# Desperodoo/distributed_multi_agent_reinforcement_learning

Measured on AMD Instinct MI355X. Metric: env-steps/sec (whole node), pursuit-evasion 8-agent 4096-env, higher is better.
Workload: dtype f64 environment / f32 policy (f32 matrix products evaluated from exact 3-way bf16 operand splits, f32 accumulation and storage)

## Files before the change

### distributed_multi_agent_reinforcement_learning_amd/csrc/mappo_ops.hip

```cpp
#include <hip/hip_runtime.h>
#include <stdint.h>
#include <stdlib.h>
#include <string.h>

#include <mutex>

#include "mappo_ops.h"
#include "mappo_ops_diag.h"
#include "sb_common.hpp"
#include "sb_wgrad.hpp"

namespace {

constexpr int MAX_P = 16;

__device__ __forceinline__ float msg_dot4(const float *w, const float4 &qv) {
    return __builtin_fmaf(w[3], qv.w, __builtin_fmaf(w[2], qv.z, __builtin_fmaf(w[1], qv.y, w[0] * qv.x)));
}

struct MsgDims {
    int R, P, K, E, din, q_div, adj_mode, rpb;
    int64_t p_rs, q_rs, e_rs, adj_rs, o_is;
};

// ... 750 lines not shown
    stats[2] = mean;
    stats[3] = sqrt(var > 0.0 ? var : 0.0);
}

__global__ __launch_bounds__(256) void k_gae_center(int64_t n, const float *adv, double *stats) {
    const double mean = stats[2];
    double d = 0.0, unused = 0.0;
    for (int64_t i = (int64_t)blockIdx.x * 256 + threadIdx.x; i < n; i += (int64_t)gridDim.x * 256) {
        const double x = (double)adv[i] - mean;
        d += x * x;
    }
    gae_block_sum(d, unused);
    if (threadIdx.x == 0) stats[4 + 2 * blockIdx.x] = d;
}

__global__ void k_gae_std(int64_t n, int nblk, double *stats) {
    double d = 0.0;
    for (int b = 0; b < nblk; b++) d += stats[4 + 2 * b];
    stats[1] = d;
    stats[3] = sqrt(d / (double)(n - 1));
}

__global__ void k_gae_norm(int64_t n, float *adv, const float *active, const double *stats) {
    const int64_t i = (int64_t)blockIdx.x * blockDim.x + threadIdx.x;
    if (i < n) {
        const float mean = (float)stats[2], sd = (float)stats[3];
        adv[i] = (adv[i] - mean) / (sd + 1e-5f) * active[i];
    }
}

__global__ void k_advance_counter(uint64_t *ctr, uint64_t by) { *ctr += by; }

constexpr int SN_MAX_A = 16, SN_MAX_H = 1024;
__global__ __launch_bounds__(256) void k_sn_power(int A, int H, const float *__restrict__ W, float *u, float *v, float eps, int n_iter,
                                                  float *__restrict__ w_eff) {
    __shared__ float s_u[SN_MAX_A], s_s[SN_MAX_A], s_v[SN_MAX_H], s_red[4];
    const int tid = threadIdx.x, lane = tid & 63, wave = tid >> 6;
    if (tid < A) s_u[tid] = u[tid];
    for (int k = tid; k < H; k += 256) s_v[k] = v[k];
    __syncthreads();
    for (int it = 0; it <= n_iter; it++) {
        if (it > 0) {
            float part = 0.f;
            for (int k = tid; k < H; k += 256) {
                float t = 0.f;
                for (int a = 0; a < A; a++) t = __builtin_fmaf(W[(size_t)a * H + k], s_u[a], t);
                s_v[k] = t;
                part = __builtin_fmaf(t, t, part);
            }
            for (int off = 32; off > 0; off >>= 1) part += __shfl_xor(part, off);
            if (lane == 0) s_red[wave] = part;
            __syncthreads();
            const float den = fmaxf(sqrtf((s_red[0] + s_red[1]) + (s_red[2] + s_red[3])), eps);
            for (int k = tid; k < H; k += 256) s_v[k] = s_v[k] / den;
            __syncthreads();
        }
        for (int a = wave; a < A; a += 4) {
            float part = 0.f;
            for (int k = lane; k < H; k += 64) part = __builtin_fmaf(W[(size_t)a * H + k], s_v[k], part);
            for (int off = 32; off > 0; off >>= 1) part += __shfl_xor(part, off);
            if (lane == 0) s_s[a] = part;
        }
        __syncthreads();
        if (it > 0) {
            if (tid == 0) {
                float q = 0.f;
                for (int a = 0; a < A; a++) q = __builtin_fmaf(s_s[a], s_s[a], q);
                const float den = fmaxf(sqrtf(q), eps);
                for (int a = 0; a < A; a++) s_u[a] = s_s[a] / den;
            }
            __syncthreads();
        }
    }
    float sigma = 0.f;
    for (int a = 0; a < A; a++) sigma = __builtin_fmaf(s_u[a], s_s[a], sigma);
    for (int i = tid; i < A * H; i += 256) w_eff[i] = W[i] / sigma;
    if (n_iter > 0) {
        if (tid < A) u[tid] = s_u[tid];
        for (int k = tid; k < H; k += 256) v[k] = s_v[k];
    }
}

__device__ __forceinline__ void philox4x32_10(uint32_t c0, uint32_t c1, uint32_t c2, uint32_t c3, uint32_t k0, uint32_t k1, uint32_t *o) {
    for (int i = 0; i < 10; i++) {
        const uint64_t p0 = (uint64_t)0xD2511F53u * c0, p1 = (uint64_t)0xCD9E8D57u * c2;
        const uint32_t n0 = (uint32_t)(p1 >> 32) ^ c1 ^ k0, n1 = (uint32_t)p1, n2 = (uint32_t)(p0 >> 32) ^ c3 ^ k1, n3 = (uint32_t)p0;
        c0 = n0; c1 = n1; c2 = n2; c3 = n3;
        k0 += 0x9E3779B9u; k1 += 0xBB67AE85u;
    }
    o[0] = c0; o[1] = c1; o[2] = c2; o[3] = c3;
}

__global__ void k_categorical(int R, int A, const float *probs, uint64_t seed, uint64_t offset, const uint64_t *offset_dev, int greedy,
                              int32_t *action, float *logp) {
    const int r = blockIdx.x * blockDim.x + threadIdx.x;
    if (r >= R) return;
    if (offset_dev) offset += *offset_dev;
    const float *p = probs + (size_t)r * A;
    float tot = 0.f;
    for (int k = 0; k < A; k++) tot += p[k];
    int a = 0;
    if (greedy) {
        float best = p[0];
        for (int k = 1; k < A; k++) if (p[k] > best) { best = p[k]; a = k; }
    } else {
        uint32_t o[4];
        const uint64_t ctr = offset + (uint64_t)r;
        philox4x32_10((uint32_t)ctr, (uint32_t)(ctr >> 32), 0u, 0u, (uint32_t)seed, (uint32_t)(seed >> 32), o);
// ... 3 lines not shown
        for (int k = 0; k < A; k++) {
            cum += p[k];
            if (p[k] > 0.f) a = k;
            if (u < cum) break;
        }
    }
    action[r] = a;
    if (logp) {
        float pn = p[a] / tot;
        pn = fminf(fmaxf(pn, 1.1920929e-07f), 1.f - 1.1920929e-07f);
        logp[r] = logf(pn);
    }
}


__device__ __forceinline__ void wave_fence() {
    __builtin_amdgcn_fence(__ATOMIC_RELEASE, "wavefront");
    __builtin_amdgcn_wave_barrier();
    __builtin_amdgcn_fence(__ATOMIC_ACQUIRE, "wavefront");
}

template <int CTRL>
__device__ __forceinline__ float dpp_f(float v) { return __int_as_float(__builtin_amdgcn_update_dpp(0, __float_as_int(v), CTRL, 0xF, 0xF, true)); }
__device__ __forceinline__ float row16_sum(float v) {
    v += dpp_f<0xB1>(v);
    v += dpp_f<0x4E>(v);
    v += dpp_f<0x141>(v);
    v += dpp_f<0x140>(v);
    return v;
}

constexpr int HEAD_MAX_A = 16, HEAD_H = 128;
template <bool SAMPLE, int AT>
__global__ __launch_bounds__(256) void k_head(int R, int A, const float *__restrict__ feat, const float *__restrict__ W, const float *__restrict__ b,
                                              float *__restrict__ y, uint64_t seed, uint64_t *counter, unsigned int *done, int greedy,
                                              int32_t *__restrict__ action, float *__restrict__ logp) {
    __shared__ float s_y[4][64][AT + 1];
    const int lane = threadIdx.x & 63, wave = threadIdx.x >> 6, nw = (gridDim.x * blockDim.x) >> 6;
    const int i = lane & 15, g = lane >> 4;
    float w[AT][8];
#pragma unroll
    for (int a = 0; a < AT; a++)
#pragma unroll
        for (int k = 0; k < 8; k++) w[a][k] = W[a * HEAD_H + 8 * i + k];
    const uint64_t offset = SAMPLE ? *counter : 0ull;
    float (*sy)[AT + 1] = s_y[wave];
    for (int r0 = (blockIdx.x * 4 + wave) * 64; r0 < R; r0 += nw * 64) {
        float4 fall[16][2];
#pragma unroll
        for (int st = 0; st < 16; st++) {
            const int r = r0 + 4 * st + g;
            fall[st][0] = fall[st][1] = make_float4(0.f, 0.f, 0.f, 0.f);
            if (r < R) {
                fall[st][0] = *(const float4 *)(feat + (size_t)r * HEAD_H + 8 * i);
                fall[st][1] = *(const float4 *)(feat + (size_t)r * HEAD_H + 8 * i + 4);
            }
        }
#pragma unroll
        for (int st = 0; st < 16; st++) {
            const int row = 4 * st + g;
            const float4 fa = fall[st][0], fb = fall[st][1];
            float mine = 0.f;
#pragma unroll
            for (int a = 0; a < AT; a++) {
                float sum = fa.x * w[a][0];
                sum = __builtin_fmaf(fa.y, w[a][1], sum); sum = __builtin_fmaf(fa.z, w[a][2], sum); sum = __builtin_fmaf(fa.w, w[a][3], sum);
                sum = __builtin_fmaf(fb.x, w[a][4], sum); sum = __builtin_fmaf(fb.y, w[a][5], sum); sum = __builtin_fmaf(fb.z, w[a][6], sum);
                sum = __builtin_fmaf(fb.w, w[a][7], sum);
                sum = row16_sum(sum);
                mine = i == a ? sum : mine;
            }
            if (i < AT) sy[row][i] = mine;
        }
        wave_fence();
        const int r = r0 + lane;
        if (r < R) {
            float v[AT];
#pragma unroll
            for (int a = 0; a < AT; a++) v[a] = sy[lane][a] + b[a];
// ... 11 lines not shown
#pragma unroll
                for (int a = 0; a < AT; a++) { p[a] = p[a] / den; tot += p[a]; }
                int act = 0;
                float pa = p[0];
                if (greedy) {
#pragma unroll
                    for (int a = 1; a < AT; a++) { const bool up = p[a] > pa; pa = up ? p[a] : pa; act = up ? a : act; }
                } else {
                    uint32_t o[4];
                    const uint64_t ctr = offset + (uint64_t)r;
                    philox4x32_10((uint32_t)ctr, (uint32_t)(ctr >> 32), 0u, 0u, (uint32_t)seed, (uint32_t)(seed >> 32), o);
                    const float u = ((float)(o[0] >> 8) + 0.5f) * (1.0f / 16777216.0f) * tot;
                    float cum = 0.f;
                    bool found = false;
                    act = AT - 1;
                    pa = p[AT - 1];
#pragma unroll
                    for (int a = 0; a < AT; a++) {
                        cum += p[a];
                        const bool take = !found && p[a] > 0.f;
                        act = take ? a : act;
                        pa = take ? p[a] : pa;
                        found = found || u < cum;
                    }
                }
                action[r] = act;
                float pn = pa / tot;
                pn = fminf(fmaxf(pn, 1.1920929e-07f), 1.f - 1.1920929e-07f);
                logp[r] = logf(pn);
            }
        }
        wave_fence();
    }
    if (SAMPLE) {
        __syncthreads();
        if (threadIdx.x == 0) {
            __threadfence();
            if (atomicAdd(done, 1u) == gridDim.x - 1) {
                *counter = offset + (uint64_t)R;
                *done = 0u;
                __threadfence();
            }
        }
    }
}

__device__ __forceinline__ float sigmoidf_(float x) { return 1.f / (1.f + expf(-x)); }
__device__ __forceinline__ float sigmoid_hw(float x) { return __builtin_amdgcn_rcpf(1.f + __expf(-x)); }
__device__ __forceinline__ float tanh_hw(float x) { return 1.f - 2.f * __builtin_amdgcn_rcpf(1.f + __expf(2.f * x)); }

__global__ void k_gru_gates_fwd(int B, int H, const float *gi, const float *gh, const float *bhh, const float *hprev, float *hout,
                                float *save ) {
    const int idx = blockIdx.x * blockDim.x + threadIdx.x;
    const int H4 = H >> 2;
    if (idx >= B * H4) return;
    const int b = idx / H4, c = (idx - b * H4) << 2;
    const float4 gir = *(const float4 *)(gi + (size_t)b * 3 * H + c), giz = *(const float4 *)(gi + (size_t)b * 3 * H + H + c),
                 gin = *(const float4 *)(gi + (size_t)b * 3 * H + 2 * H + c);
    const float4 ghr = *(const float4 *)(gh + (size_t)b * 3 * H + c), ghz = *(const float4 *)(gh + (size_t)b * 3 * H + H + c),
                 ghn = *(const float4 *)(gh + (size_t)b * 3 * H + 2 * H + c);
    const float4 br = *(const float4 *)(bhh + c), bz = *(const float4 *)(bhh + H + c), bn = *(const float4 *)(bhh + 2 * H + c);
    const float4 hp = *(const float4 *)(hprev + (size_t)b * H + c);
    float4 r, z, n, hn, ho;
#define GRU_ONE(f)                                  \
    r.f = sigmoidf_(gir.f + ghr.f + br.f);          \
    z.f = sigmoidf_(giz.f + ghz.f + bz.f);          \
    hn.f = ghn.f + bn.f;                            \
    n.f = tanhf(gin.f + r.f * hn.f);                \
    ho.f = (1.f - z.f) * n.f + z.f * hp.f;
    GRU_ONE(x) GRU_ONE(y) GRU_ONE(z) GRU_ONE(w)
#undef GRU_ONE
    *(float4 *)(hout + (size_t)b * H + c) = ho;
    if (save) {
        const size_t BH = (size_t)B * H, o = (size_t)b * H + c;
        *(float4 *)(save + o) = r; *(float4 *)(save + BH + o) = z; *(float4 *)(save + 2 * BH + o) = n; *(float4 *)(save + 3 * BH + o) = hn;
    }
// ... 1307 lines not shown

int head_grid(int R) { const int g = (R + 255) / 256; return g < 1024 ? g : 1024; }

int head_linear(int32_t R, int32_t A, int32_t H, const float *feat, const float *W, const float *b, float *y, void *stream) {
    if (R < 0 || A < 1 || A > HEAD_MAX_A || H != HEAD_H || !feat || !W || !b || !y || ((uintptr_t)feat & 15)) return MO_ERR_BAD_ARG;
    if (R == 0) return 0;
    hipStream_t st = (hipStream_t)stream;
#define HEAD_LIN(AT) case AT: hipLaunchKernelGGL((k_head<false, AT>), dim3(head_grid(R)), dim3(256), 0, st, R, A, feat, W, b, y, (uint64_t)0, \
                                       (uint64_t *)nullptr, (unsigned int *)nullptr, 0, (int32_t *)nullptr, (float *)nullptr); break;
    switch (A) {
        HEAD_LIN(1) HEAD_LIN(2) HEAD_LIN(3) HEAD_LIN(4) HEAD_LIN(5) HEAD_LIN(6) HEAD_LIN(7) HEAD_LIN(8) HEAD_LIN(9) HEAD_LIN(10) HEAD_LIN(11)
        HEAD_LIN(12) HEAD_LIN(13) HEAD_LIN(14) HEAD_LIN(15) HEAD_LIN(16)
    }
#undef HEAD_LIN
    return (int)hipGetLastError();
}

int head_sample(int32_t R, int32_t A, int32_t H, const float *feat, const float *W, const float *b, uint64_t seed, uint64_t *counter,
                uint32_t *ticket, int32_t greedy, int32_t *action, float *logp, void *stream) {
    if (R < 0 || A < 1 || A > HEAD_MAX_A || H != HEAD_H || !feat || !W || !b || !counter || !ticket || !action || !logp || ((uintptr_t)feat & 15))
        return MO_ERR_BAD_ARG;
    if (R == 0) return 0;
    hipStream_t st = (hipStream_t)stream;
#define HEAD_SMP(AT) case AT: hipLaunchKernelGGL((k_head<true, AT>), dim3(head_grid(R)), dim3(256), 0, st, R, A, feat, W, b, (float *)nullptr, seed, \
                                       counter, ticket, (int)greedy, action, logp); break;
    switch (A) {
        HEAD_SMP(1) HEAD_SMP(2) HEAD_SMP(3) HEAD_SMP(4) HEAD_SMP(5) HEAD_SMP(6) HEAD_SMP(7) HEAD_SMP(8) HEAD_SMP(9) HEAD_SMP(10) HEAD_SMP(11)
        HEAD_SMP(12) HEAD_SMP(13) HEAD_SMP(14) HEAD_SMP(15) HEAD_SMP(16)
    }
#undef HEAD_SMP
    return (int)hipGetLastError();
}

int gru_gates_fwd(int32_t B, int32_t H, const float *gi, const float *gh, const float *b_hh, const float *h_prev, float *h_out,
                  float *save, void *stream) {
    if (B < 1 || H < 4 || (H & 3) || !gi || !gh || !b_hh || !h_prev || !h_out) return MO_ERR_BAD_ARG;
    const int n = B * (H >> 2);
    hipLaunchKernelGGL(k_gru_gates_fwd, dim3((n + 255) / 256), dim3(256), 0, (hipStream_t)stream, B, H, gi, gh, b_hh, h_prev, h_out, save);
    return (int)hipGetLastError();
}

int gru_gates_bwd(int32_t B, int32_t H, const float *dout, const float *dcarry, const float *save, const float *h_prev, float *dgi,
                  float *dgh, float *dh_direct, void *stream) {
    if (B < 1 || H < 4 || (H & 3) || !save || !h_prev || !dgi || !dgh || !dh_direct) return MO_ERR_BAD_ARG;
    const int n = B * (H >> 2);
    hipLaunchKernelGGL(k_gru_gates_bwd, dim3((n + 255) / 256), dim3(256), 0, (hipStream_t)stream, B, H, dout, dcarry, save, h_prev, dgi, dgh,
                       dh_direct);
    return (int)hipGetLastError();
}

int gru_cell_fwd_multi(int32_t n_nets, const mo_gru_cell_net *nets, int32_t B, int32_t H, void *stream) {
    if (n_nets < 1 || n_nets > MO_GRU_CELL_MAX_NETS || !nets || B < 1 || H != GRU_H) return MO_ERR_BAD_ARG;
    GruCellNets a;
    memset(&a, 0, sizeof a);
    for (int k = 0; k < n_nets; k++) {
        const mo_gru_cell_net &m = nets[k];
        if (!m.x || !m.h_prev || !m.w_ih || !m.w_hh || !m.b_ih || !m.b_hh || !m.h_out) return MO_ERR_BAD_ARG;
        if (((uintptr_t)m.x & 15) || ((uintptr_t)m.h_prev & 15) || ((uintptr_t)m.w_ih & 15) || ((uintptr_t)m.w_hh & 15)) return MO_ERR_BAD_ARG;
        a.n[k] = m;
    }
    const int nblk = (B + GRU_RB - 1) / GRU_RB;
    int dev = 0, cus = 256;
    if (hipGetDevice(&dev) == hipSuccess && hipDeviceGetAttribute(&cus, hipDeviceAttributeMultiprocessorCount, dev) != hipSuccess) cus = 256;
    int per = cus / n_nets;
    if (per < 1) per = 1;
    const int grid = nblk < per ? nblk : per;
// ... 284 lines not shown
```

### distributed_multi_agent_reinforcement_learning_amd/mappo.py

```python
import contextlib
import gc
import logging
import threading
import types

import numpy as np
import torch

from . import ops
from .model import build_actor_critic, pair_embeddings, pair_heads, sequence_forward_pair
from .pe_env import status_or, status_text

_log = logging.getLogger(__name__)

BUFFER_KEYS = ("p_state", "e_state", "o_state", "p_adj", "e_adj", "o_adj", "actor_historical_embedding",
               "critic_historical_embedding", "v_n", "a_n", "a_logprob_n", "r", "active")


class _Buffer(dict):

    def __missing__(self, key):
        if key == "o_adj" and "o_adj_bits" in self:
            v = ops.unpack_adj_bits(self["o_adj_bits"], self.num_obstacle_slots)
            self[key] = v
# ... 404 lines not shown
        _gc_depth += 1
    try:
        yield
    finally:
        with _gc_lock:
            _gc_depth -= 1
            if _gc_depth == 0 and _gc_was_on:
                gc.enable()


class _RolloutState:

    def __init__(self, agent, env):
        self.agent = agent
        N, P = env.num_envs, env.num_defender
        O = env.pe_cfg.O
        d, L, H, E = agent.depth, agent.num_layers, agent.rnn_hidden_dim, agent.embedding_dim
        dev = agent.device
        self.N, self.P, self.d = N, P, d
        z = lambda *s: torch.zeros(s, dtype=torch.float32, device=dev)
        self.obs = dict(p_state=z(N, P, 4), e_state=z(N, 1, 4), p_adj=z(N, P, P), e_adj=z(N, P, 1),
                        o_adj_bits=torch.zeros((N, P, ops.adj_row_words(O)), dtype=torch.int32, device=dev))
        self.o_state = z(N, O, 4)
        self.o_kvalid = torch.zeros(N, dtype=torch.int32, device=dev)
        self.hbuf_a, self.hbuf_c = z(2, L, N * P, H), z(2, L, N * P, H)
        self.quirk = bool(agent.reference_quirks and agent.actor.shared_net is agent.critic.shared_net)
        self.M = ((d + 1) // 2 if self.quirk else d) + 1
        self.ring = z(self.M, 2, N, P, E)
        self.t = 0
        self.a_n = torch.zeros((N, P), dtype=torch.int32, device=dev)
        self.logp, self.v, self.raw = z(N, P), z(N, P), z(N, P)
        self.counter = torch.full((1,), int(agent.sample_rank) << 40, dtype=torch.int64, device=dev)
        self.ticket = torch.zeros(1, dtype=torch.int32, device=dev)
        self.period = self.M if self.M % 2 == 0 else 2 * self.M
        self.graphs = {}
        self.pair_forward = agent.actor.shared_net is agent.critic.shared_net
        ops.gemm_workspace(dev)

    @property
    def ha(self):
        return self.hbuf_a[self.t & 1]

    @property
    def hc(self):
        return self.hbuf_c[self.t & 1]

    @property
    def a_cur(self):
        return self.ring[(self.t - 1) % self.M][0]

    @property
    def c_cur(self):
        return self.ring[(self.t - 1) % self.M][1]

    @property
    def hist_c(self):
        return None if self.quirk else self.ring[:, 1]

    def reset(self, env):
        for t in (self.hbuf_a, self.hbuf_c, self.ring):
            t.zero_()
        self.t = 0
        self.o_state.copy_(env.boundary_map.obstacle_agent)
        self.o_kvalid.copy_(env.n_obs)

    def _obs(self):
        o = dict(self.obs)
        o["o_state"], o["o_kvalid"] = self.o_state, self.o_kvalid
        return o

    def _hops(self, t):
        d, M, ring = self.d, self.M, self.ring
        if self.quirk:
            hops = [ring[(t - 1 - j // 2) % M][1 - j % 2] for j in range(d)]
            return hops, hops
        return [ring[(t - 1 - k) % M][0] for k in range(d)], [ring[(t - 1 - k) % M][1] for k in range(d)]

    def policy_step(self, forced_actions=None):
        ag = self.agent
        hops_a, hops_c = self._hops(self.t)
        slot = self.ring[self.t % self.M]
        a_cur, c_cur = slot[0], slot[1]
        o = self._obs()
        ha_cur, hc_cur = self.ha, self.hc
        ha_new, hc_new = self.hbuf_a[(self.t + 1) & 1], self.hbuf_c[(self.t + 1) & 1]
        if self.pair_forward and not torch.is_grad_enabled():
            emb = ag.actor.shared_net.forward_pair(o["p_state"], o["e_state"], o["o_state"], o["p_adj"], o["e_adj"], o["o_adj_bits"],
                                                   hops_a, hops_c, o["o_kvalid"], 1, slot)
            a_emb, c_emb = emb[0], emb[1]
            if ag.actor.use_rnn and ag.critic.use_rnn:
                E = a_emb.shape[-1]
                fa, fc = ops.gru_step_multi([a_emb.reshape(-1, E), c_emb.reshape(-1, E)], [ha_cur, hc_cur], [ag.actor.GRU, ag.critic.GRU],
                                            hiddens_out=[ha_new, hc_new])
                feat_a, feat_c = fa.reshape(self.N, self.P, -1), fc.reshape(self.N, self.P, -1)
                ha, hc = ha_new, hc_new
            else:
                feat_a, ha = ag.actor._rollout_features(a_emb, ha_cur, True)
                feat_c, hc = ag.critic._rollout_features(c_emb, hc_cur, True)
            v = ag.critic.head(feat_c, out=self.v)
            w_a = ag.actor.head_weight() if forced_actions is None else None
            feat_a = feat_a.contiguous()
            if w_a is not None and ops._head_ok(feat_a, w_a, ag.actor.Mean.bias):
                ops.head_sample(feat_a, w_a, ag.actor.Mean.bias, ag.sample_seed, self.counter, self.ticket, (self.a_n, self.logp))
                prob = None
            else:
                prob = torch.softmax(ag.actor.head(feat_a), dim=-1)
        else:
            prob, ha, a_emb = ag.actor(o, hops_a, ha_cur, 0, inplace_hidden=True, emb_out=a_cur)
            v, hc, c_emb = ag.critic(o, hops_c, hc_cur, 0, rollout=True, inplace_hidden=True, emb_out=c_cur)
        if forced_actions is not None:
            self.a_n.copy_(forced_actions.to(torch.int32))
            self.logp.copy_(torch.distributions.Categorical(probs=prob).log_prob(forced_actions))
        elif prob is not None:
            ops.categorical_sample(prob, ag.sample_seed, 0, counter=self.counter, out=(self.a_n, self.logp))
        if ha is not ha_new:
            ha_new.copy_(ha)
        if hc is not hc_new:
            hc_new.copy_(hc)
        if a_emb.data_ptr() != a_cur.data_ptr():
            a_cur.copy_(a_emb)
        if c_emb.data_ptr() != c_cur.data_ptr():
            c_cur.copy_(c_emb)
        if v.data_ptr() != self.v.data_ptr():
            self.v.copy_(v.reshape(self.N, self.P))

    def step(self, forced_actions=None):
        self.policy_step(forced_actions)
        self.t += 1

    def value_step(self):
        ag, d, t, M = self.agent, self.d, self.t, self.M
        hops = []
        if d:
            if self.quirk:
                hops = ([self.ring[(t - 1) % M][1]] + self._hops(t - 1)[1])[:d]
            else:
                hops = self._hops(t)[1]
        v, hc, c_emb = ag.critic(self._obs(), hops, self.hc, 0, rollout=True)
        self.v.copy_(v.reshape(self.N, self.P))

    def replay_policy_step(self):
        phase = self.t % self.period
        g = self.graphs.get(phase)
        if g is None:
            g = self.graphs[phase] = self._capture()
        g.replay()
        self.t += 1

    def _capture(self):
        live = (self.hbuf_a, self.hbuf_c, self.ring, self.counter, self.a_n, self.logp, self.v)
        keep = [t.clone() for t in live]
        side = torch.cuda.Stream()
        side.wait_stream(torch.cuda.current_stream())
        with torch.cuda.stream(side):
            for _ in range(2):
                self.policy_step()
        torch.cuda.current_stream().wait_stream(side)
        g = torch.cuda.CUDAGraph()
        with _collector_paused():
            with torch.cuda.graph(g, capture_error_mode="thread_local"):
                self.policy_step()
        for t, k in zip(live, keep):
            t.copy_(k)
        return g
```

### distributed_multi_agent_reinforcement_learning_amd/model.py

```python
import torch
import torch.nn as nn
import torch.nn.functional as F
from torch.nn.utils import spectral_norm
from torch.nn.utils.spectral_norm import SpectralNorm

from . import ops


class HeadLinear(nn.Linear):

    def forward(self, x):
        return ops.linear_skinny(x, self.weight, self.bias)


def _ortho_linear(n_in, n_out, cls=nn.Linear):
    layer = cls(n_in, n_out)
    for name, param in layer.named_parameters():
        if "bias" in name:
            nn.init.constant_(param, 0)
        elif "weight" in name:
            nn.init.orthogonal_(param, gain=1.0)
    return layer


# ... 128 lines not shown
                h = cats[k + 1][..., E:]
            else:
                h = out if out is not None else torch.empty((2, R, P, E), dtype=p.dtype, device=p.device)
            cat_2d, h_2d = cats[k].view(2 * R * P, 2 * E), ops.block2d(h)
            if ops.split_linear_ok(cat_2d, fk.weight, h_2d):
                ops.split_linear(cat_2d, fk.weight, fk.bias, True, out=h_2d)
            else:
                ops.gemm_nt(cat_2d, fk.weight, fk.bias, True, out=h_2d)
        return h


def _o_adj(obs):
    return obs["o_adj_bits"] if "o_adj_bits" in obs else obs["o_adj"]


class _Trunk(nn.Module):
    use_rnn = True

    def _rollout_features(self, embedding, hidden_state, inplace_hidden=False):
        R, P, E = embedding.shape
        if not self.use_rnn:
            return embedding, hidden_state
        feat, hidden_state = ops.gru(embedding.reshape(1, R * P, E), hidden_state, self.GRU, inplace_hidden)
        return feat.reshape(R, P, self.rnn_hidden_dim), hidden_state

    def _sequence_features(self, embedding, batch, steps):
        P = embedding.shape[1]
        if not self.use_rnn:
            return embedding.reshape(batch, steps, P, self.rnn_input_dim).permute(1, 0, 2, 3)
        h0 = torch.zeros(self.num_layers, batch * P, self.rnn_hidden_dim, dtype=embedding.dtype, device=embedding.device)
        feat, _ = ops.gru(embedding.reshape(batch * steps * P, self.rnn_input_dim), h0, self.GRU, agents=P, steps=steps)
        return feat.reshape(steps, batch, P, self.rnn_hidden_dim)

    def head_weight(self):
        m = self.Mean
        if torch.is_grad_enabled() or not m.bias.is_cuda:
            return None
        hooks = list(m._forward_pre_hooks.values())
        if not hooks:
            return m.weight
        if (len(hooks) == 1 and isinstance(hooks[0], SpectralNorm) and hooks[0].name == "weight" and hooks[0].dim == 0 and m.weight_orig.dim() == 2
                and m.weight_orig.shape[0] <= 16 and m.weight_orig.shape[1] <= 1024):
            return ops.spectral_norm_weight(m.weight_orig, m.weight_u, m.weight_v, hooks[0].eps,
                                            hooks[0].n_power_iterations if m.training else 0)
        return None

    def head(self, feat, out=None):
        w = self.head_weight()
        if w is None:
            y = self.Mean(feat)
            return y if out is None else out.copy_(y.reshape(out.shape))
        return ops.head_linear(feat, w, self.Mean.bias, out=out)

    def get_weights(self):
        return {k: v.cpu() for k, v in self.state_dict().items()}

    def set_weights(self, weights):
        self.load_state_dict(weights)

    def get_gradients(self):
        return [None if p.grad is None else p.grad.data.cpu().numpy() for p in self.parameters()]

    def set_gradients(self, gradients, device):
        for g, p in zip(gradients, self.parameters()):
            if g is not None:
                p.grad = torch.as_tensor(g).to(device)


class SharedActor(_Trunk):
    def __init__(self, shared_net, rnn_input_dim, action_dim, num_layers, rnn_hidden_dim, is_sn=False):
        super().__init__()
        self.shared_net = shared_net
        self.num_layers = num_layers
        self.rnn_input_dim = rnn_input_dim
        self.rnn_hidden_dim = rnn_hidden_dim
        self.GRU = nn.GRU(rnn_input_dim, rnn_hidden_dim, num_layers)
        self.Mean = _make_linear(rnn_hidden_dim, action_dim, is_sn, HeadLinear)

# ... 150 lines not shown
```

### distributed_multi_agent_reinforcement_learning_amd/ops.py

```python
import ctypes as C
import os

import torch
import torch.nn.functional as F

from . import build as _build

ADJ_TENSOR, ADJ_ONES, ADJ_VALID, ADJ_BITS = 0, 1, 2, 3
EXPORTS = ("dhgn_msg_agg_fwd", "dhgn_msg_agg3_fwd", "dhgn_msg_agg_bwd", "dhgn_msg_agg_bwd_workspace", "dhgn_msg_agg_ones_sorted_ok", "dhgn_msg_agg_ones_sorted_fwd",
           "dhgn_msg_agg_ones_sorted_bwd", "dhgn_msg_agg_ones_sorted_workspace", "gae_advnorm", "gae_advnorm_workspace", "categorical_sample",
           "categorical_sample_counter",
           "gru_gates_fwd", "gru_gates_bwd", "gru_cell_fwd", "gru_cell_fwd_multi", "gru_cell_split_fwd_multi", "sb_gemm_n128", "sb_gemm", "gru_seq_fwd", "gru_seq_fwd_multi", "gru_seq_split_fwd_multi", "gru_seq_split_bwd_multi", "gru_seq_save_elems", "gru_seq_bwd", "gru_seq_bwd_multi", "gru_seq_bwd_workspace", "wgrad_tn", "wgrad_tn_workspace", "wgrad_split_tn", "wgrad_split_tn2", "wgrad_split_workspace", "rollout_record", "ppo_loss_fwd_bwd", "ppo_loss_prob_fwd_bwd", "ppo_loss_workspace",
           "gauss_head_sample", "ppo_loss_gauss_fwd_bwd", "ppo_loss_gauss_workspace", "gauss_head_sample_ex", "ppo_loss_gauss_ex_fwd_bwd",
           "ppo_loss_gauss_ex_workspace", "mappo_ops_error_string")

_lib = None


def lib_path():
    return _build.lib_path("libmappo_ops.so")


def load_library():
    global _lib
    if _lib is None:
        path = lib_path()
        if not os.path.exists(path):
            raise RuntimeError(f"{path} is missing: build it with __graft_entry__.build() (hipcc --offload-arch=gfx950); "
                               "the fused MAPPO ops have no fallback")
        L = C.CDLL(path)
        vp, i32, i64, f32 = C.c_void_p, C.c_int32, C.c_int64, C.c_float
        L.dhgn_msg_agg_fwd.argtypes = [i32, i32, i32, i32, i32, vp, i64, vp, i64, i32, vp, i64, vp, i64, i32, vp, vp, vp, vp, i64, vp]
        L.dhgn_msg_agg_bwd.argtypes = [i32, i32, i32, i32, i32, vp, i64, vp, i64, i32, vp, i64, vp, i64, i32, vp, vp, vp, vp, i64, vp, vp, vp, vp]
        L.dhgn_msg_agg3_fwd.argtypes = [vp, i32, i32, i32, vp, i64, vp, i64, vp]
        L.dhgn_msg_agg3_pair_fwd.argtypes = [vp, i32, i32, i32, vp, i64, vp, vp, vp, i64, vp]
        L.dhgn_msg_agg3_pair01_fwd.argtypes = [vp, i32, i32, i32, vp, i64, vp, vp, i64, vp]
        L.dhgn_msg_agg_bwd_pair.argtypes = [i32, i32, i32, i32, i32, vp, i64, vp, i64, i32, vp, i64, vp, i64, vp, vp, vp, vp, i64, vp, vp, vp, vp]
        L.dhgn_msg_agg3_pair_pos_fwd.argtypes = [vp, i32, i32, i32, vp, i64, vp, vp, vp, i64, vp, i64, vp, vp, vp, i64, vp]
        L.spectral_norm_weight.argtypes = [i32, i32, vp, vp, vp, f32, i32, vp, vp]
        L.dhgn_msg_agg_bwd_workspace.argtypes = [i32, i32]
        L.dhgn_msg_agg_bwd_workspace.restype = i64
        L.dhgn_msg_agg_ones_sorted_ok.argtypes = [i32] * 6
        L.dhgn_msg_agg_ones_sorted_workspace.argtypes = [i32, i32, i32, i32, i32, vp, vp, vp]
        L.dhgn_msg_agg_ones_sorted_workspace.restype = i64
        L.dhgn_msg_agg_ones_sorted_fwd.argtypes = [i32, i32, i32, i32, vp, i64, vp, i64, i32, vp, vp, vp, i64, vp, vp, vp]
        L.dhgn_msg_agg_ones_sorted_bwd.argtypes = [i32, i32, i32, i32, vp, i64, i32, vp, i64, vp, vp, vp, vp, vp, vp]
        L.gae_advnorm.argtypes = [i32, i32, i32, vp, vp, vp, f32, f32, i32, vp, vp, vp, vp]
        L.gae_advnorm_workspace.restype = i64
        L.categorical_sample.argtypes = [i32, i32, vp, C.c_uint64, C.c_uint64, i32, vp, vp, vp]
        L.categorical_sample_counter.argtypes = [i32, i32, vp, C.c_uint64, vp, i32, vp, vp, vp]
        L.head_linear.argtypes = [i32, i32, i32, vp, vp, vp, vp, vp]
        L.head_sample.argtypes = [i32, i32, i32, vp, vp, vp, C.c_uint64, vp, vp, i32, vp, vp, vp]
        L.gru_gates_fwd.argtypes = [i32, i32, vp, vp, vp, vp, vp, vp, vp]
        L.gru_gates_bwd.argtypes = [i32, i32, vp, vp, vp, vp, vp, vp, vp, vp]
        L.gru_cell_fwd.argtypes = [i32, i32, vp, vp, vp, vp, vp, vp, vp, vp]
        L.gru_seq_fwd.argtypes = [i32, i32, i32, vp, vp, vp, vp, vp, vp, i32, vp]
        L.gru_seq_bwd.argtypes = [i32, i32, i32, vp, vp, vp, vp, vp, vp, vp, vp, vp, vp, vp, i32, vp, vp]
        L.gru_cell_fwd_multi.argtypes = [i32, vp, i32, i32, vp]
        L.gru_cell_split_fwd_multi.argtypes = [i32, vp, i32, i32, vp]
        L.sb_gemm_n128.argtypes = [i64, i32, vp, i64, vp, i64, vp, i32, vp, i64, vp, i64, vp]
        L.sb_gemm.argtypes = [i64, i32, i32, vp, i64, vp, i64, vp, i32, vp, i64, vp, i64, vp]
        L.gru_seq_fwd_multi.argtypes = [i32, vp, i32, i32, i32, i32, vp]
        L.gru_seq_bwd_multi.argtypes = [i32, vp, i32, i32, i32, i32, vp]
        L.gru_seq_split_fwd_multi.argtypes = [i32, vp, i32, i32, i32, i32, vp]
        L.gru_seq_split_bwd_multi.argtypes = [i32, vp, i32, i32, i32, i32, vp]
        L.gru_seq_save_elems.argtypes = [i32, i32]
        L.gru_seq_save_elems.restype = i64
        L.gru_seq_bwd_workspace.argtypes = [i32]
        L.gru_seq_bwd_workspace.restype = i64
        L.wgrad_tn_workspace.argtypes = [i32, i32]
        L.wgrad_tn_workspace.restype = i64
        L.wgrad_tn.argtypes = [i64, i32, i32, vp, i64, vp, i64, vp, i32, vp, vp]
        L.wgrad_split_workspace.restype = i64
        L.wgrad_split_workspace.argtypes = [i32, i32]
        L.wgrad_split_tn.argtypes = [i64, i32, i32, vp, i64, vp, i64, vp, i32, vp, vp]
        L.wgrad_split_tn2.argtypes = [i64, i32, i32, i32, vp, i64, vp, i64, vp, i64, vp, i32, vp, vp]
        L.fcra_neighbour_mean.argtypes = [i32, i32, i32, i32, vp, i64, i64, vp, i64, i64, vp, i64, vp, i32, vp, vp, i64, vp]
        L.fcra_neighbour_mean_multi.argtypes = [i32, vp, i32, i32, i32, i32, i64, i64, i64, i64, vp, i64, i32, i64, vp]
        L.sb_gemm_signs.argtypes = [i64, i32, i32, vp, i64, vp, i64, vp, i32, vp, i64, vp, i64, vp, i64, vp]
        L.sb_gemm_masked_bits.argtypes = [i64, i32, i32, vp, i64, vp, i64, vp, i64, i32, vp, i64, vp, vp, vp]
        L.sb_gemm_masked_workspace.argtypes = [i32]
        L.sb_gemm_masked_workspace.restype = i64
        L.sb_gemm_masked.argtypes = [i64, i32, i32, vp, i64, vp, i64, vp, i64, i32, vp, i64, vp, vp, vp]
        L.relu_bwd_colsum_workspace.argtypes = [i32]
        L.relu_bwd_colsum_workspace.restype = i64
# ... 418 lines not shown
    return (feat.is_cuda and feat.dtype == torch.float32 and feat.is_contiguous() and W.shape[1] == HEAD_FEATURES and feat.shape[-1] == HEAD_FEATURES
            and W.shape[0] <= HEAD_MAX_OUT and b is not None and not torch.is_grad_enabled()
            and feat.data_ptr() % 16 == 0)


def head_linear(feat, W, b, out=None):
    if not _head_ok(feat, W, b):
        y = F.linear(feat, W, b)
        return y if out is None else out.copy_(y.reshape(out.shape))
    L = load_library()
    A = W.shape[0]
    R = feat.numel() // HEAD_FEATURES
    if out is None:
        out = torch.empty(feat.shape[:-1] + (A,), dtype=torch.float32, device=feat.device)
    assert out.is_contiguous() and out.numel() == R * A and out.dtype == torch.float32
    _check(L.head_linear(R, A, HEAD_FEATURES, _ptr(feat), _ptr(W.detach().contiguous()), _ptr(b.detach().contiguous()), _ptr(out), _stream()),
           "head_linear")
    return out


def head_sample(feat, W, b, seed, counter, ticket, out, greedy=False):
    assert _head_ok(feat, W, b)
    L = load_library()
    action, logp = out
    R = feat.numel() // HEAD_FEATURES
    assert action.dtype == torch.int32 and logp.dtype == torch.float32 and action.is_contiguous() and logp.is_contiguous()
    assert action.numel() == R and logp.numel() == R and counter.dtype == torch.int64 and counter.numel() == 1
    assert ticket.dtype == torch.int32 and ticket.numel() == 1
    _check(L.head_sample(R, W.shape[0], HEAD_FEATURES, _ptr(feat), _ptr(W.detach().contiguous()), _ptr(b.detach().contiguous()), int(seed),
                         _ptr(counter), _ptr(ticket), 1 if greedy else 0, _ptr(action), _ptr(logp), _stream()), "head_sample")
    return action, logp


def gauss_head_sample(feat, W, b, log_std, seed, counter, ticket, out, greedy=False):
    assert _head_ok(feat, W, b) and log_std.shape == (W.shape[0],)
    L = load_library()
    action, env_action, logp = out
    A, R = W.shape[0], feat.numel() // HEAD_FEATURES
    assert action.dtype == torch.float32 and env_action.dtype == torch.float64 and logp.dtype == torch.float32
    assert all(t.is_contiguous() for t in out) and action.numel() == R * A and env_action.numel() == R * A and logp.numel() == R
    assert counter.dtype == torch.int64 and counter.numel() == 1 and ticket.dtype == torch.int32 and ticket.numel() == 1
    _check(L.gauss_head_sample(R, A, HEAD_FEATURES, _ptr(feat), _ptr(W.detach().contiguous()), _ptr(b.detach().contiguous()),
                               _ptr(log_std.detach().contiguous()), int(seed), _ptr(counter), _ptr(ticket), 1 if greedy else 0, _ptr(action),
                               _ptr(env_action), _ptr(logp), _stream()), "gauss_head_sample")
    return action, env_action, logp


GAUSS_SQUASH = {"clip": 0, "tanh": 1}


def gauss_head_sample_ex(feat, W, b, log_std, seed, counter, ticket, out, greedy=False, log_std_min=-float("inf"), log_std_max=float("inf"),
                         squash="clip"):
    state = isinstance(log_std, (tuple, list))
    A = W.shape[0]
    assert _head_ok(feat, W, b) and squash in GAUSS_SQUASH
    if state:
        W_ls, b_ls = (t.detach().contiguous() for t in log_std)
        assert W_ls.shape == W.shape and b_ls.shape == (A,) and W_ls.dtype == b_ls.dtype == torch.float32 and A <= 8
        ls = None
    else:
        assert log_std.shape == (A,)
        W_ls = b_ls = None
        ls = log_std.detach().contiguous()
    L = load_library()
    action, env_action, logp = out
    R = feat.numel() // HEAD_FEATURES
# ... 1081 lines not shown
```

### include/mappo_ops.h

```cpp
#ifndef MAPPO_OPS_H
#define MAPPO_OPS_H
#include <stdint.h>

#ifdef __cplusplus
extern "C" {
#endif

#define MO_ERR_BAD_ARG 20001

enum { MO_ADJ_TENSOR = 0,
       MO_ADJ_ONES = 1,
       MO_ADJ_VALID = 2,
       MO_ADJ_BITS = 3 };
#define MO_ADJ_ROW_WORDS(K) (((((K) + 31) >> 5) + 3) & ~3)

int dhgn_msg_agg_fwd(int32_t R, int32_t P, int32_t K, int32_t E, int32_t din, const float *p, int64_t p_row_stride,
                     const float *q, int64_t q_row_stride, int32_t q_div, const float *e, int64_t e_row_stride, const void *adj,
                     int64_t adj_row_stride, int32_t adj_mode, const int32_t *kvalid, const float *W, const float *b,
                     float *out, int64_t out_stride , void *stream);

typedef struct mo_msg_rel {
    int32_t K, din, q_div, adj_mode;
    const float *q; int64_t q_rs;
    const float *e; int64_t e_rs;
// ... 17 lines not shown
                               int64_t wp_row_stride, const float *bp, float *pos_actor, float *pos_critic, int64_t pos_stride, void *stream);

int64_t dhgn_msg_agg_bwd_workspace(int32_t E, int32_t din);
int dhgn_msg_agg_bwd(int32_t R, int32_t P, int32_t K, int32_t E, int32_t din, const float *p, int64_t p_row_stride,
                     const float *q, int64_t q_row_stride, int32_t q_div, const float *e, int64_t e_row_stride, const void *adj,
                     int64_t adj_row_stride, int32_t adj_mode, const int32_t *kvalid, const float *W, const float *b,
                     const float *gout, int64_t gout_stride, float *dW, float *db, void *workspace, void *stream);

int dhgn_msg_agg_ones_sorted_ok(int32_t R, int32_t P, int32_t K, int32_t E, int32_t din, int32_t q_div);
int64_t dhgn_msg_agg_ones_sorted_workspace(int32_t R, int32_t P, int32_t K, int32_t E, int32_t q_div, int64_t *m_bytes, int64_t *qtab_bytes,
                                           int64_t *partial_bytes);
int dhgn_msg_agg_ones_sorted_fwd(int32_t R, int32_t P, int32_t K, int32_t E, const float *p, int64_t p_row_stride, const float *q,
                                 int64_t q_row_stride, int32_t q_div, const float *W, const float *b, float *out, int64_t out_stride,
                                 uint8_t *save_m, float *qtab, void *stream);
int dhgn_msg_agg_ones_sorted_bwd(int32_t R, int32_t P, int32_t K, int32_t E, const float *p, int64_t p_row_stride, int32_t q_div,
                                 const float *gout, int64_t gout_stride, const uint8_t *save_m, const float *qtab, float *dW, float *db,
                                 void *partials, void *stream);

int64_t gae_advnorm_workspace(void);
int gae_advnorm(int32_t N, int32_t T, int32_t P, const float *r, const float *v, const float *active, float gamma,
                float lamda, int32_t use_adv_norm, float *adv, float *v_target, double *stats, void *stream);

int categorical_sample(int32_t R, int32_t A, const float *probs, uint64_t seed, uint64_t offset, int32_t greedy,
                       int32_t *action, float *logp, void *stream);
int categorical_sample_counter(int32_t R, int32_t A, const float *probs, uint64_t seed, uint64_t *counter, int32_t greedy,
                               int32_t *action, float *logp, void *stream);

int spectral_norm_weight(int32_t A, int32_t H, const float *W, float *u, float *v, float eps, int32_t n_power_iterations, float *w_eff,
                         void *stream);

int head_linear(int32_t R, int32_t A, int32_t H, const float *feat, const float *W, const float *b, float *y, void *stream);
int head_sample(int32_t R, int32_t A, int32_t H, const float *feat, const float *W, const float *b, uint64_t seed, uint64_t *counter,
                uint32_t *ticket, int32_t greedy, int32_t *action, float *logp, void *stream);

int gru_gates_fwd(int32_t B, int32_t H, const float *gi, const float *gh, const float *b_hh, const float *h_prev, float *h_out,
                  float *save, void *stream);
int gru_gates_bwd(int32_t B, int32_t H, const float *dout, const float *dcarry, const float *save, const float *h_prev, float *dgi,
                  float *dgh, float *dh_direct, void *stream);

int64_t gru_seq_save_elems(int32_t T, int32_t B);
#define MO_GRU_MAX_NETS 24
#define MO_GRU_CELL_MAX_NETS 4
typedef struct mo_gru_seq_net { const float *gi, *w_hh, *b_hh, *h0; float *out, *save; int32_t B, pad0; } mo_gru_seq_net;
typedef struct mo_gru_seq_bwd_net {
    const float *dout, *save, *out, *h0, *w_hh;
    float *dgi, *dgh, *dnr, *dh0, *db_ih, *db_hh;
    void *workspace;
    int32_t B, pad0;
} mo_gru_seq_bwd_net;
int gru_seq_fwd_multi(int32_t n_nets, const mo_gru_seq_net *nets, int32_t T, int32_t B, int32_t H, int32_t gi_agents, void *stream);
int gru_seq_bwd_multi(int32_t n_nets, const mo_gru_seq_bwd_net *nets, int32_t T, int32_t B, int32_t H, int32_t gi_agents, void *stream);
int gru_seq_split_fwd_multi(int32_t n_nets, const mo_gru_seq_net *nets, int32_t T, int32_t B, int32_t H, int32_t gi_agents, void *stream);
int gru_seq_split_bwd_multi(int32_t n_nets, const mo_gru_seq_bwd_net *nets, int32_t T, int32_t B, int32_t H, int32_t gi_agents, void *stream);
int gru_seq_fwd(int32_t T, int32_t B, int32_t H, const float *gi, const float *w_hh, const float *b_hh, const float *h0, float *out,
                float *save, int32_t gi_agents, void *stream);
int64_t gru_seq_bwd_workspace(int32_t B);
int gru_seq_bwd(int32_t T, int32_t B, int32_t H, const float *dout, const float *save, const float *out, const float *h0,
                const float *w_hh, float *dgi, float *dgh, float *dnr, float *dh0, float *db_ih, float *db_hh, int32_t gi_agents,
                void *workspace, void *stream);

int gru_cell_fwd(int32_t B, int32_t H, const float *x, const float *h_prev, const float *w_ih, const float *w_hh, const float *b_ih,
                 const float *b_hh, float *h_out, void *stream);
typedef struct mo_gru_cell_net { const float *x, *h_prev, *w_ih, *w_hh, *b_ih, *b_hh; float *h_out; } mo_gru_cell_net;
int gru_cell_fwd_multi(int32_t n_nets, const mo_gru_cell_net *nets, int32_t B, int32_t H, void *stream);
int gru_cell_split_fwd_multi(int32_t n_nets, const mo_gru_cell_net *nets, int32_t B, int32_t H, void *stream);
int sb_gemm_n128(int64_t R, int32_t K, const float *X, int64_t ldx, const float *W, int64_t ldw, const float *bias, int32_t relu, const float *C,
// ... 83 lines not shown
```

Baseline: 2.683 million.

## Fuse actor sample head, critic value head and spectral norm into one kernel

Adds a k_tick_tail kernel that runs the actor categorical-sampling head and the critic value head in one launch, using a 2-D grid with blockIdx.y selecting the net. Each block recomputes the spectral-norm power iteration into LDS instead of running a separate spectral_norm_weight kernel and writing w_eff to global memory. The last block, found by a ticket, writes back u/v and advances the RNG counter. This replaces several small per-step launches inside the captured rollout graph with one, at the cost of redundant per-block power iterations and more shared memory.

```diff
diff --git a/distributed_multi_agent_reinforcement_learning_amd/csrc/mappo_ops.hip b/distributed_multi_agent_reinforcement_learning_amd/csrc/mappo_ops.hip
--- a/distributed_multi_agent_reinforcement_learning_amd/csrc/mappo_ops.hip
+++ b/distributed_multi_agent_reinforcement_learning_amd/csrc/mappo_ops.hip
@@ -806,9 +806,8 @@
 __global__ void k_advance_counter(uint64_t *ctr, uint64_t by) { *ctr += by; }
 
 constexpr int SN_MAX_A = 16, SN_MAX_H = 1024;
-__global__ __launch_bounds__(256) void k_sn_power(int A, int H, const float *__restrict__ W, float *u, float *v, float eps, int n_iter,
-                                                  float *__restrict__ w_eff) {
-    __shared__ float s_u[SN_MAX_A], s_s[SN_MAX_A], s_v[SN_MAX_H], s_red[4];
+__device__ __forceinline__ float sn_power_lds(int A, int H, const float *__restrict__ W, const float *u, const float *v, float eps, int n_iter,
+                                              float *s_u, float *s_s, float *s_v, float *s_red) {
     const int tid = threadIdx.x, lane = tid & 63, wave = tid >> 6;
     if (tid < A) s_u[tid] = u[tid];
     for (int k = tid; k < H; k += 256) s_v[k] = v[k];
@@ -848,6 +847,14 @@
     }
     float sigma = 0.f;
     for (int a = 0; a < A; a++) sigma = __builtin_fmaf(s_u[a], s_s[a], sigma);
+    return sigma;
+}
+
+__global__ __launch_bounds__(256) void k_sn_power(int A, int H, const float *__restrict__ W, float *u, float *v, float eps, int n_iter,
+                                                  float *__restrict__ w_eff) {
+    __shared__ float s_u[SN_MAX_A], s_s[SN_MAX_A], s_v[SN_MAX_H], s_red[4];
+    const int tid = threadIdx.x;
+    const float sigma = sn_power_lds(A, H, W, u, v, eps, n_iter, s_u, s_s, s_v, s_red);
     for (int i = tid; i < A * H; i += 256) w_eff[i] = W[i] / sigma;
     if (n_iter > 0) {
         if (tid < A) u[tid] = s_u[tid];
@@ -917,10 +924,9 @@
 
 constexpr int HEAD_MAX_A = 16, HEAD_H = 128;
 template <bool SAMPLE, int AT>
-__global__ __launch_bounds__(256) void k_head(int R, int A, const float *__restrict__ feat, const float *__restrict__ W, const float *__restrict__ b,
-                                              float *__restrict__ y, uint64_t seed, uint64_t *counter, unsigned int *done, int greedy,
-                                              int32_t *__restrict__ action, float *__restrict__ logp) {
-    __shared__ float s_y[4][64][AT + 1];
+__device__ __forceinline__ void head_rows(int R, const float *__restrict__ feat, const float *__restrict__ W, const float *__restrict__ b,
+                                          float *__restrict__ y, uint64_t seed, uint64_t offset, int greedy, int32_t *__restrict__ action,
+                                          float *__restrict__ logp, float (*sy)[AT + 1]) {
     const int lane = threadIdx.x & 63, wave = threadIdx.x >> 6, nw = (gridDim.x * blockDim.x) >> 6;
     const int i = lane & 15, g = lane >> 4;
     float w[AT][8];
@@ -928,8 +934,6 @@
     for (int a = 0; a < AT; a++)
 #pragma unroll
         for (int k = 0; k < 8; k++) w[a][k] = W[a * HEAD_H + 8 * i + k];
-    const uint64_t offset = SAMPLE ? *counter : 0ull;
-    float (*sy)[AT + 1] = s_y[wave];
     for (int r0 = (blockIdx.x * 4 + wave) * 64; r0 < R; r0 += nw * 64) {
         float4 fall[16][2];
 #pragma unroll
@@ -1007,6 +1011,15 @@
         }
         wave_fence();
     }
+}
+
+template <bool SAMPLE, int AT>
+__global__ __launch_bounds__(256) void k_head(int R, int A, const float *__restrict__ feat, const float *__restrict__ W, const float *__restrict__ b,
+                                              float *__restrict__ y, uint64_t seed, uint64_t *counter, unsigned int *done, int greedy,
+                                              int32_t *__restrict__ action, float *__restrict__ logp) {
+    __shared__ float s_y[4][64][AT + 1];
+    const uint64_t offset = SAMPLE ? *counter : 0ull;
+    head_rows<SAMPLE, AT>(R, feat, W, b, y, seed, offset, greedy, action, logp, s_y[threadIdx.x >> 6]);
     if (SAMPLE) {
         __syncthreads();
         if (threadIdx.x == 0) {
@@ -1017,6 +1030,59 @@
                 __threadfence();
             }
         }
+    }
+}
+
+struct TailArgs {
+    mo_tail_head net[2];
+    int R;
+    uint64_t seed, *counter;
+    unsigned int *tickets;
+    int greedy;
+    int32_t *action;
+    float *logp, *value;
+};
+
+template <int AT>
+__global__ __launch_bounds__(256) void k_tick_tail(TailArgs a) {
+    constexpr int AMAX = AT > 1 ? AT : 1;
+    __shared__ float s_y[4 * 64 * (AMAX + 1)], s_w[AMAX * HEAD_H], s_u[SN_MAX_A], s_s[SN_MAX_A], s_v[HEAD_H], s_red[4];
+    __shared__ int s_last;
+    const int tid = threadIdx.x, wave = tid >> 6;
+    const bool critic = blockIdx.y != 0;
+    const mo_tail_head &h = a.net[critic ? 1 : 0];
+    const int A = critic ? 1 : AT;
+    const float *W = h.W;
+    if (h.sn_u) {
+        const float sigma = sn_power_lds(A, HEAD_H, h.W, h.sn_u, h.sn_v, h.sn_eps, h.sn_iters, s_u, s_s, s_v, s_red);
+        for (int i = tid; i < A * HEAD_H; i += 256) s_w[i] = h.W[i] / sigma;
+        __syncthreads();
+        W = s_w;
+    }
+    uint64_t offset = 0ull;
+    if (critic) {
+        head_rows<false, 1>(a.R, h.feat, W, h.b, a.value, 0ull, 0ull, 0, nullptr, nullptr, (float (*)[2])(s_y + wave * 64 * 2));
+    } else {
+        offset = *a.counter;
+        head_rows<true, AT>(a.R, h.feat, W, h.b, nullptr, a.seed, offset, a.greedy, a.action, a.logp, (float (*)[AT + 1])(s_y + wave * 64 * (AT + 1)));
+    }
+    const bool power = h.sn_u && h.sn_iters > 0;
+    if (critic && !power) return;
+    __syncthreads();
+    if (tid == 0) {
+        __threadfence();
+        s_last = atomicAdd(a.tickets + (critic ? 1 : 0), 1u) == gridDim.x - 1;
+    }
+    __syncthreads();
+    if (!s_last) return;
+    if (power) {
+        if (tid < A) h.sn_u[tid] = s_u[tid];
+        for (int k = tid; k < HEAD_H; k += 256) h.sn_v[k] = s_v[k];
+    }
+    if (tid == 0) {
+        if (!critic) *a.counter = offset + (uint64_t)a.R;
+        a.tickets[critic ? 1 : 0] = 0u;
+        __threadfence();
     }
 }
 
@@ -2390,6 +2456,30 @@
     return (int)hipGetLastError();
 }
 
+int tick_tail(int32_t R, int32_t A, int32_t H, const mo_tail_head *actor, const mo_tail_head *critic, uint64_t seed, uint64_t *counter,
+              uint32_t *tickets, int32_t greedy, int32_t *action, float *logp, float *value, void *stream) {
+    if (R < 0 || A < 1 || A > HEAD_MAX_A || H != HEAD_H || !actor || !critic || !counter || !tickets || !action || !logp || !value)
+        return MO_ERR_BAD_ARG;
+    TailArgs a;
+    memset(&a, 0, sizeof a);
+    a.net[0] = *actor;
+    a.net[1] = *critic;
+    for (int k = 0; k < 2; k++) {
+        const mo_tail_head &h = a.net[k];
+        if (!h.feat || !h.W || !h.b || ((uintptr_t)h.feat & 15) || (!h.sn_u != !h.sn_v) || (h.sn_u && h.sn_iters < 0)) return MO_ERR_BAD_ARG;
+    }
+    if (R == 0) return 0;
+    a.R = R; a.seed = seed; a.counter = counter; a.tickets = tickets; a.greedy = greedy; a.action = action; a.logp = logp; a.value = value;
+    hipStream_t st = (hipStream_t)stream;
+#define TICK_TAIL(AT) case AT: hipLaunchKernelGGL((k_tick_tail<AT>), dim3(head_grid(R), 2), dim3(256), 0, st, a); break;
+    switch (A) {
+        TICK_TAIL(1) TICK_TAIL(2) TICK_TAIL(3) TICK_TAIL(4) TICK_TAIL(5) TICK_TAIL(6) TICK_TAIL(7) TICK_TAIL(8) TICK_TAIL(9) TICK_TAIL(10) TICK_TAIL(11)
+        TICK_TAIL(12) TICK_TAIL(13) TICK_TAIL(14) TICK_TAIL(15) TICK_TAIL(16)
+    }
+#undef TICK_TAIL
+    return (int)hipGetLastError();
+}
+
 int gru_gates_fwd(int32_t B, int32_t H, const float *gi, const float *gh, const float *b_hh, const float *h_prev, float *h_out,
                   float *save, void *stream) {
     if (B < 1 || H < 4 || (H & 3) || !gi || !gh || !b_hh || !h_prev || !h_out) return MO_ERR_BAD_ARG;
diff --git a/distributed_multi_agent_reinforcement_learning_amd/mappo.py b/distributed_multi_agent_reinforcement_learning_amd/mappo.py
--- a/distributed_multi_agent_reinforcement_learning_amd/mappo.py
+++ b/distributed_multi_agent_reinforcement_learning_amd/mappo.py
@@ -460,6 +460,7 @@
         self.logp, self.v, self.raw = z(N, P), z(N, P), z(N, P)
         self.counter = torch.full((1,), int(agent.sample_rank) << 40, dtype=torch.int64, device=dev)
         self.ticket = torch.zeros(1, dtype=torch.int32, device=dev)
+        self.tail_tickets = torch.zeros(2, dtype=torch.int32, device=dev)
         self.period = self.M if self.M % 2 == 0 else 2 * self.M
         self.graphs = {}
         self.pair_forward = agent.actor.shared_net is agent.critic.shared_net
@@ -525,14 +526,20 @@
             else:
                 feat_a, ha = ag.actor._rollout_features(a_emb, ha_cur, True)
                 feat_c, hc = ag.critic._rollout_features(c_emb, hc_cur, True)
-            v = ag.critic.head(feat_c, out=self.v)
-            w_a = ag.actor.head_weight() if forced_actions is None else None
             feat_a = feat_a.contiguous()
-            if w_a is not None and ops._head_ok(feat_a, w_a, ag.actor.Mean.bias):
-                ops.head_sample(feat_a, w_a, ag.actor.Mean.bias, ag.sample_seed, self.counter, self.ticket, (self.a_n, self.logp))
-                prob = None
+            fused = (ops.TICK_TAIL and forced_actions is None and ag.actor.use_rnn and ag.critic.use_rnn and ops.CELL_MODE == "split_bf16")
+            spec_a, spec_c = (ag.actor.head_spec(), ag.critic.head_spec()) if fused else (None, None)
+            if spec_a is not None and spec_c is not None and ops.tick_tail_ok(feat_a, feat_c, spec_a, spec_c):
+                ops.tick_tail(feat_a, feat_c, spec_a, spec_c, ag.sample_seed, self.counter, self.tail_tickets, (self.a_n, self.logp, self.v))
+                v, prob = self.v, None
             else:
-                prob = torch.softmax(ag.actor.head(feat_a), dim=-1)
+                v = ag.critic.head(feat_c, out=self.v)
+                w_a = ag.actor.head_weight() if forced_actions is None else None
+                if w_a is not None and ops._head_ok(feat_a, w_a, ag.actor.Mean.bias):
+                    ops.head_sample(feat_a, w_a, ag.actor.Mean.bias, ag.sample_seed, self.counter, self.ticket, (self.a_n, self.logp))
+                    prob = None
+                else:
+                    prob = torch.softmax(ag.actor.head(feat_a), dim=-1)
         else:
             prob, ha, a_emb = ag.actor(o, hops_a, ha_cur, 0, inplace_hidden=True, emb_out=a_cur)
             v, hc, c_emb = ag.critic(o, hops_c, hc_cur, 0, rollout=True, inplace_hidden=True, emb_out=c_cur)
@@ -568,7 +575,7 @@
         self.v.copy_(v.reshape(self.N, self.P))
 
     def replay_policy_step(self):
-        phase = self.t % self.period
+        phase = (self.t % self.period, ops.TICK_TAIL)
         g = self.graphs.get(phase)
         if g is None:
             g = self.graphs[phase] = self._capture()
diff --git a/distributed_multi_agent_reinforcement_learning_amd/model.py b/distributed_multi_agent_reinforcement_learning_amd/model.py
--- a/distributed_multi_agent_reinforcement_learning_amd/model.py
+++ b/distributed_multi_agent_reinforcement_learning_amd/model.py
@@ -184,18 +184,24 @@
         feat, _ = ops.gru(embedding.reshape(batch * steps * P, self.rnn_input_dim), h0, self.GRU, agents=P, steps=steps)
         return feat.reshape(steps, batch, P, self.rnn_hidden_dim)
 
-    def head_weight(self):
+    def head_spec(self):
         m = self.Mean
         if torch.is_grad_enabled() or not m.bias.is_cuda:
             return None
         hooks = list(m._forward_pre_hooks.values())
         if not hooks:
-            return m.weight
+            return m.weight, m.bias, None, None, 0.0, 0
         if (len(hooks) == 1 and isinstance(hooks[0], SpectralNorm) and hooks[0].name == "weight" and hooks[0].dim == 0 and m.weight_orig.dim() == 2
                 and m.weight_orig.shape[0] <= 16 and m.weight_orig.shape[1] <= 1024):
-            return ops.spectral_norm_weight(m.weight_orig, m.weight_u, m.weight_v, hooks[0].eps,
-                                            hooks[0].n_power_iterations if m.training else 0)
+            return m.weight_orig, m.bias, m.weight_u, m.weight_v, hooks[0].eps, hooks[0].n_power_iterations if m.training else 0
         return None
+
+    def head_weight(self):
+        spec = self.head_spec()
+        if spec is None:
+            return None
+        W, _, u, v, eps, iters = spec
+        return W if u is None else ops.spectral_norm_weight(W, u, v, eps, iters)
 
     def head(self, feat, out=None):
         w = self.head_weight()
diff --git a/distributed_multi_agent_reinforcement_learning_amd/ops.py b/distributed_multi_agent_reinforcement_learning_amd/ops.py
--- a/distributed_multi_agent_reinforcement_learning_amd/ops.py
+++ b/distributed_multi_agent_reinforcement_learning_amd/ops.py
@@ -10,7 +10,7 @@
 EXPORTS = ("dhgn_msg_agg_fwd", "dhgn_msg_agg3_fwd", "dhgn_msg_agg_bwd", "dhgn_msg_agg_bwd_workspace", "dhgn_msg_agg_ones_sorted_ok", "dhgn_msg_agg_ones_sorted_fwd",
            "dhgn_msg_agg_ones_sorted_bwd", "dhgn_msg_agg_ones_sorted_workspace", "gae_advnorm", "gae_advnorm_workspace", "categorical_sample",
            "categorical_sample_counter",
-           "gru_gates_fwd", "gru_gates_bwd", "gru_cell_fwd", "gru_cell_fwd_multi", "gru_cell_split_fwd_multi", "sb_gemm_n128", "sb_gemm", "gru_seq_fwd", "gru_seq_fwd_multi", "gru_seq_split_fwd_multi", "gru_seq_split_bwd_multi", "gru_seq_save_elems", "gru_seq_bwd", "gru_seq_bwd_multi", "gru_seq_bwd_workspace", "wgrad_tn", "wgrad_tn_workspace", "wgrad_split_tn", "wgrad_split_tn2", "wgrad_split_workspace", "rollout_record", "ppo_loss_fwd_bwd", "ppo_loss_prob_fwd_bwd", "ppo_loss_workspace",
+           "gru_gates_fwd", "gru_gates_bwd", "gru_cell_fwd", "gru_cell_fwd_multi", "gru_cell_split_fwd_multi", "sb_gemm_n128", "sb_gemm", "gru_seq_fwd", "gru_seq_fwd_multi", "gru_seq_split_fwd_multi", "gru_seq_split_bwd_multi", "gru_seq_save_elems", "gru_seq_bwd", "gru_seq_bwd_multi", "gru_seq_bwd_workspace", "wgrad_tn", "wgrad_tn_workspace", "wgrad_split_tn", "wgrad_split_tn2", "wgrad_split_workspace", "rollout_record", "tick_tail", "ppo_loss_fwd_bwd", "ppo_loss_prob_fwd_bwd", "ppo_loss_workspace",
            "gauss_head_sample", "ppo_loss_gauss_fwd_bwd", "ppo_loss_gauss_workspace", "gauss_head_sample_ex", "ppo_loss_gauss_ex_fwd_bwd",
            "ppo_loss_gauss_ex_workspace", "mappo_ops_error_string")
 
@@ -51,6 +51,7 @@
         L.categorical_sample_counter.argtypes = [i32, i32, vp, C.c_uint64, vp, i32, vp, vp, vp]
         L.head_linear.argtypes = [i32, i32, i32, vp, vp, vp, vp, vp]
         L.head_sample.argtypes = [i32, i32, i32, vp, vp, vp, C.c_uint64, vp, vp, i32, vp, vp, vp]
+        L.tick_tail.argtypes = [i32, i32, i32, vp, vp, C.c_uint64, vp, vp, i32, vp, vp, vp, vp]
         L.gru_gates_fwd.argtypes = [i32, i32, vp, vp, vp, vp, vp, vp, vp]
         L.gru_gates_bwd.argtypes = [i32, i32, vp, vp, vp, vp, vp, vp, vp, vp]
         L.gru_cell_fwd.argtypes = [i32, i32, vp, vp, vp, vp, vp, vp, vp, vp]
@@ -535,6 +536,45 @@
     return action, logp
 
 
+TICK_TAIL = os.environ.get("MAPPO_TICK_TAIL", "1") != "0"
+
+
+class TailHead(C.Structure):
+    _fields_ = [(n, C.c_void_p) for n in ("feat", "W", "b", "sn_u", "sn_v")] + [("sn_eps", C.c_float), ("sn_iters", C.c_int32)]
+
+
+def _tail_head(feat, spec, keep):
+    W, b, u, v, eps, iters = spec
+    W, b = W.detach().contiguous(), b.detach().contiguous()
+    keep += [W, b]
+    h = TailHead()
+    h.feat, h.W, h.b = feat.data_ptr(), W.data_ptr(), b.data_ptr()
+    if u is not None:
+        assert u.is_contiguous() and v.is_contiguous() and u.shape == (W.shape[0],) and v.shape == (HEAD_FEATURES,) and u.dtype == v.dtype == torch.float32
+        h.sn_u, h.sn_v, h.sn_eps, h.sn_iters = u.data_ptr(), v.data_ptr(), float(eps), int(iters)
+    return h
+
+
+def tick_tail_ok(feat_a, feat_c, spec_a, spec_c):
+    return (_head_ok(feat_a, spec_a[0], spec_a[1]) and _head_ok(feat_c, spec_c[0], spec_c[1]) and spec_c[0].shape[0] == 1
+            and feat_a.numel() == feat_c.numel() and all(t.dtype == torch.float32 and t.is_cuda for t in spec_a[:2] + spec_c[:2]))
+
+
+def tick_tail(feat_a, feat_c, spec_a, spec_c, seed, counter, tickets, out, greedy=False):
+    assert tick_tail_ok(feat_a, feat_c, spec_a, spec_c)
+    L = load_library()
+    action, logp, value = out
+    R = feat_a.numel() // HEAD_FEATURES
+    assert action.dtype == torch.int32 and logp.dtype == value.dtype == torch.float32
+    assert all(t.is_contiguous() and t.numel() == R and t.is_cuda for t in out)
+    assert counter.dtype == torch.int64 and counter.numel() == 1 and tickets.dtype == torch.int32 and tickets.numel() == 2 and tickets.is_contiguous()
+    keep = []
+    ha, hc = _tail_head(feat_a, spec_a, keep), _tail_head(feat_c, spec_c, keep)
+    _check(L.tick_tail(R, spec_a[0].shape[0], HEAD_FEATURES, C.byref(ha), C.byref(hc), int(seed), _ptr(counter), _ptr(tickets),
+                       1 if greedy else 0, _ptr(action), _ptr(logp), _ptr(value), _stream()), "tick_tail")
+    return action, logp, value
+
+
 def gauss_head_sample(feat, W, b, log_std, seed, counter, ticket, out, greedy=False):
     assert _head_ok(feat, W, b) and log_std.shape == (W.shape[0],)
     L = load_library()
diff --git a/include/mappo_ops.h b/include/mappo_ops.h
--- a/include/mappo_ops.h
+++ b/include/mappo_ops.h
@@ -73,6 +73,15 @@
 int head_linear(int32_t R, int32_t A, int32_t H, const float *feat, const float *W, const float *b, float *y, void *stream);
 int head_sample(int32_t R, int32_t A, int32_t H, const float *feat, const float *W, const float *b, uint64_t seed, uint64_t *counter,
                 uint32_t *ticket, int32_t greedy, int32_t *action, float *logp, void *stream);
+
+typedef struct {
+    const float *feat, *W, *b;
+    float *sn_u, *sn_v;
+    float sn_eps;
+    int32_t sn_iters;
+} mo_tail_head;
+int tick_tail(int32_t R, int32_t A, int32_t H, const mo_tail_head *actor, const mo_tail_head *critic, uint64_t seed, uint64_t *counter,
+              uint32_t *tickets, int32_t greedy, int32_t *action, float *logp, float *value, void *stream);
 
 int gru_gates_fwd(int32_t B, int32_t H, const float *gi, const float *gh, const float *b_hh, const float *h_prev, float *h_out,
                   float *save, void *stream);
```

Result: no change. 2.695 million (median of 6 runs) (+0.4%).
